# helenypzhang/Subspace-Multimodal-Learning

Measured on AMD Instinct MI355X. Metric: bags/sec fwd+bwd, DeformCrossTransMIL N=10k x 512, higher is better.
Workload: dtype f32

## Files before the change

### include/smml.h

```cpp
#ifndef SMML_H_
#define SMML_H_

#include <stddef.h>

#define SMML_ABI_VERSION 2

#ifdef __cplusplus
extern "C" {
#endif

const char* smml_last_error(void);
int smml_abi_version(void);
int smml_device_check(int device);
void* smml_event_create(void);
int smml_event_destroy(void* ev);
int smml_event_record(void* ev, void* stream);
int smml_event_elapsed_ms(void* start, void* stop, float* ms);

int smml_gemm_f32(const float* A, const float* B, float* C, const float* bias, const float* residual,
                  int M, int N, int K, long long sam, long long sak, long long sbk, long long sbn,
                  long long ldc, long long ldr, int nb0, int nb1, long long sa0, long long sa1,
                  long long sb0, long long sb1, long long sc0, long long sc1, long long sbias0,
                  long long sbias1, int bias_mode, int rows_per_bias, long long bias_ld, int act,
                  int splitk, int accumulate, float alpha, float beta, void* stream);
size_t smml_gemm_f32_det_workspace_bytes(int M, int N, int nb0, int nb1, int splitk);
int smml_gemm_f32_det(const float* A, const float* B, float* C, const float* bias, const float* residual,
                      int M, int N, int K, long long sam, long long sak, long long sbk, long long sbn,
                      long long ldc, long long ldr, int nb0, int nb1, long long sa0, long long sa1,
                      long long sb0, long long sb1, long long sc0, long long sc1, long long sbias0,
                      long long sbias1, int bias_mode, int rows_per_bias, long long bias_ld, int act,
                      int splitk, int accumulate, float alpha, float beta, void* workspace, size_t workspace_bytes,
                      void* stream);
void smml_gemm_force_generic(int on);
void smml_gemm_set_mode(int mode);
int smml_gemm_get_mode(void);
void smml_gemm_set_small_tile(int v);

int smml_gemm_b16(const void* A, const void* B, void* C, const float* bias, int M, int N, int K, long long lda, long long ldb,
                  long long ldc, int trans, int out_bf16, int splitk, void* stream);
void smml_gemm_b16_set_tile(int mode);
void smml_gemm_b16_set_slice_major(int on);
int smml_gemm_b16_batched(const void* A, const void* B, void* C, const float* bias, int M, int N, int K, long long lda, long long ldb,
                          long long ldc, int trans, int out_bf16, int splitk, int nb, long long sa, long long sb, long long sc, void* stream);

int smml_grouped_pointwise_applies(int groups, int cin_g, int cout_g);
int smml_grouped_pointwise_fwd_f32(const float* x, const float* w, float* y, long long rows, int groups, int cin_g, int cout_g, void* stream);
int smml_grouped_pointwise_dx_f32(const float* dy, const float* w, float* dx, long long rows, int groups, int cin_g, int cout_g, void* stream);
size_t smml_grouped_pointwise_dw_workspace_bytes(long long rows, int groups, int cin_g, int cout_g);
int smml_grouped_pointwise_dw_f32(const float* dy, const float* x, float* dw, long long rows, int groups, int cin_g, int cout_g,
                                  void* workspace, size_t workspace_bytes, void* stream);

int smml_layernorm_fwd_f32(const float* x, const float* gamma, const float* beta, float* y, float* mean,
                           float* rstd, long long R, int C, float eps, void* stream);
int smml_layernorm_bwd_f32(const float* x, const float* dy, const float* gamma, const float* mean,
                           const float* rstd, float* dx, float* dgamma, float* dbeta, long long R, int C,
                           long long rows_per_dy, float dy_scale, int accumulate_dx, void* stream);
size_t smml_layernorm_bwd_det_workspace_bytes(long long R, int C);
int smml_layernorm_bwd_det_f32(const float* x, const float* dy, const float* gamma, const float* mean,
                               const float* rstd, float* dx, float* dgamma, float* dbeta, long long R, int C,
                               long long rows_per_dy, float dy_scale, int accumulate_dx, void* workspace,
                               size_t workspace_bytes, void* stream);

int smml_colsum_f32(const float* x, float* out, int nb, long long R, int C, float scale, void* stream);
size_t smml_colsum_det_workspace_bytes(int nb, long long R, int C);
int smml_colsum_det_f32(const float* x, float* out, int nb, long long R, int C, float scale, void* workspace,
                        size_t workspace_bytes, void* stream);

int smml_orth_loss_f32(const float* P, const float* Ph, const float* G, const float* Gh, const float* dloss, float* loss,
                       float* dP, float* dPh, float* dG, float* dGh, int B, int D, float gamma, void* stream);

int smml_batchloss_tail_f32(const float* go, const float* gv, const float* dloss, float* loss, float* dgo, float* dgv, int R, int nv,
                            float n_total, void* stream);

int smml_relu_bwd_f32(const float* dy, const float* y, float* dx, long long n, void* stream);

int smml_offsets_out_len(int s, int ks, int r);
int smml_offsets_fwd_f32(const float* q, const float* w0, const float* b0, const float* w2, float* vgrid,
                         float* vs, int B, int Hh, int Ww, int G, int dg, int ks, int r, int posdim,
                         float offset_scale, void* stream);
size_t smml_offsets_bwd_workspace_bytes(int B, int Hh, int Ww, int G, int dg, int ks, int r, int posdim);
int smml_offsets_bwd_f32(const float* q, const float* w0, const float* b0, const float* w2,
                         const float* dvgrid, const float* dvs, float* dq, float* dw0, float* db0,
                         float* dw2, void* workspace, size_t workspace_bytes, int B, int Hh, int Ww, int G, int dg,
                         int ks, int r, int posdim, float offset_scale, int accumulate_dq, void* stream);

int smml_bilinear_sample_fwd_f32(const float* x, const float* vs, float* kv, int B, int Hh, int Ww, int G,
// ... 260 lines not shown
```

### subspace-multimodal-learning_amd/csrc/rowops.hip

```cpp
#include <algorithm>
#include "smml_common.h"

namespace {

constexpr int MAXV = 16;

__global__ __launch_bounds__(256) void layernorm_fwd_kernel(const float* __restrict__ x, const float* __restrict__ gamma,
                                                            const float* __restrict__ beta, float* __restrict__ y,
                                                            float* __restrict__ mean, float* __restrict__ rstd, long long R,
                                                            int C, float eps) {
  const int lane = threadIdx.x & 63;
  const long long row = (long long)blockIdx.x * 4 + (threadIdx.x >> 6);
  if (row >= R) return;
  const float* xr = x + row * C;
  float v[MAXV];
  float s = 0.f;
  const int nv = (C + 63) >> 6;
#pragma unroll
  for (int i = 0; i < MAXV; ++i) {
    if (i < nv) {
      const int c = lane + 64 * i;
      v[i] = (c < C) ? xr[c] : 0.f;
      s += v[i];
    }
// ... 37 lines not shown
  const int lane = threadIdx.x & 63, wave = threadIdx.x >> 6, hl = lane & 31, half = lane >> 5;
  const bool low = hl < 16;
  const float4 gm = *reinterpret_cast<const float4*>(gamma + 4 * hl), bt = *reinterpret_cast<const float4*>(beta + 4 * hl);
  const long long stride = (long long)gridDim.x * (8 * U);
  for (long long base = ((long long)blockIdx.x * 4 + wave) * (2 * U); base < R; base += stride) {
    float4 xv[U];
#pragma unroll
    for (int u = 0; u < U; ++u) {
      const long long row = base + 2 * u + half;
      xv[u] = *reinterpret_cast<const float4*>(x + (row < R ? row : R - 1) * C + 4 * hl);
    }
#pragma unroll
    for (int u = 0; u < U; ++u) {
      const long long row = base + 2 * u + half;
      const float4 own = xv[u];
      const float4 oth = make_float4(__shfl_xor(own.x, 16), __shfl_xor(own.y, 16), __shfl_xor(own.z, 16), __shfl_xor(own.w, 16));
      const float4 lo = low ? own : oth, hi = low ? oth : own;
      const float mu = row128_sum((0.f + lo.x) + hi.x, (0.f + lo.y) + hi.y, (0.f + lo.z) + hi.z, (0.f + lo.w) + hi.w) / (float)C;
      const float4 dl = make_float4(lo.x - mu, lo.y - mu, lo.z - mu, lo.w - mu);
      const float4 dh = make_float4(hi.x - mu, hi.y - mu, hi.z - mu, hi.w - mu);
      const float ss = row128_sum(fmaf(dh.x, dh.x, dl.x * dl.x), fmaf(dh.y, dh.y, dl.y * dl.y), fmaf(dh.z, dh.z, dl.z * dl.z),
                                  fmaf(dh.w, dh.w, dl.w * dl.w));
      const float rs = rsqrtf(ss / (float)C + eps);
      if (row < R) {
        const float4 d = low ? dl : dh;
        *reinterpret_cast<float4*>(y + row * C + 4 * hl) = make_float4(fmaf(d.x * rs, gm.x, bt.x), fmaf(d.y * rs, gm.y, bt.y),
                                                                       fmaf(d.z * rs, gm.z, bt.z), fmaf(d.w * rs, gm.w, bt.w));
        if (hl == 0) { mean[row] = mu; rstd[row] = rs; }
      }
    }
  }
}

__global__ __launch_bounds__(256) void layernorm_bwd_kernel(const float* __restrict__ x, const float* __restrict__ dy,
                                                            const float* __restrict__ gamma, const float* __restrict__ mean,
                                                            const float* __restrict__ rstd, float* __restrict__ dx,
                                                            float* __restrict__ dgamma, float* __restrict__ dbeta,
                                                            long long R, int C, long long rows_per_dy, float dy_scale,
                                                            int accumulate_dx, float* __restrict__ part) {
  __shared__ float red[2][4][64 * MAXV];
  const int lane = threadIdx.x & 63, wave = threadIdx.x >> 6;
  const int nv = (C + 63) >> 6;
  float ag[MAXV], ab[MAXV], gm[MAXV];
#pragma unroll
  for (int i = 0; i < MAXV; ++i) {
    ag[i] = 0.f; ab[i] = 0.f;
    const int c = lane + 64 * i;
    gm[i] = (i < nv && c < C) ? gamma[c] : 0.f;
  }
  for (long long row = (long long)blockIdx.x * 4 + wave; row < R; row += (long long)gridDim.x * 4) {
    const float* xr = x + row * C;
    const float* dr = dy + (row / rows_per_dy) * C;
    const float mu = mean[row], rs = rstd[row];
    float xh[MAXV], gd[MAXV];
    float s1 = 0.f, s2 = 0.f;
#pragma unroll
    for (int i = 0; i < MAXV; ++i) {
      if (i < nv) {
        const int c = lane + 64 * i;
        const bool ok = c < C;
        const float d = ok ? dr[c] * dy_scale : 0.f;
        xh[i] = ok ? (xr[c] - mu) * rs : 0.f;
        gd[i] = d * gm[i];
        s1 += gd[i];
        s2 += gd[i] * xh[i];
        ag[i] += d * xh[i];
        ab[i] += d;
      }
    }
    s1 = wave_sum(s1) / (float)C;
    s2 = wave_sum(s2) / (float)C;
    float* dxr = dx + row * C;
#pragma unroll
    for (int i = 0; i < MAXV; ++i) {
      if (i < nv) {
        const int c = lane + 64 * i;
        if (c < C) {
          const float v = rs * (gd[i] - s1 - xh[i] * s2);
          dxr[c] = accumulate_dx ? dxr[c] + v : v;
        }
      }
    }
  }
#pragma unroll
  for (int i = 0; i < MAXV; ++i) {
    if (i < nv) { red[0][wave][lane + 64 * i] = ag[i]; red[1][wave][lane + 64 * i] = ab[i]; }
  }
  __syncthreads();
  for (int c = threadIdx.x; c < C; c += 256) {
    const float g = red[0][0][c] + red[0][1][c] + red[0][2][c] + red[0][3][c];
    const float b = red[1][0][c] + red[1][1][c] + red[1][2][c] + red[1][3][c];
    if (part) {
      part[((size_t)blockIdx.x * 2 + 0) * C + c] = g;
      part[((size_t)blockIdx.x * 2 + 1) * C + c] = b;
    } else {
      atomicAdd(&dgamma[c], g);
      atomicAdd(&dbeta[c], b);
    }
  }
}

__device__ __forceinline__ float half_sum(float v) {
#pragma unroll
  for (int off = 16; off > 0; off >>= 1) v += __shfl_xor(v, off);
  return v;
}

__global__ __launch_bounds__(256) void layernorm_bwd128_kernel(const float* __restrict__ x, const float* __restrict__ dy,
                                                               const float* __restrict__ gamma, const float* __restrict__ mean,
                                                               const float* __restrict__ rstd, float* __restrict__ dx,
                                                               float* __restrict__ dgamma, float* __restrict__ dbeta,
                                                               long long R, long long rows_per_dy, float dy_scale,
                                                               int accumulate_dx, float* __restrict__ part) {
  constexpr int C = 128;
  __shared__ float red[2][8][C];
  const int lane = threadIdx.x & 63, wave = threadIdx.x >> 6, hl = lane & 31, half = lane >> 5;
  const float4 gm = *reinterpret_cast<const float4*>(gamma + 4 * hl);
  float4 ag = make_float4(0.f, 0.f, 0.f, 0.f), ab = ag;
  const long long stride = (long long)gridDim.x * 16;
  for (long long r0 = ((long long)blockIdx.x * 4 + wave) * 4 + half; r0 < R; r0 += stride) {
    float4 xv[2], dv[2];
    float mu[2], rs[2];
    bool ok[2];
#pragma unroll
    for (int u = 0; u < 2; ++u) {
      const long long row = r0 + 2 * u;
      ok[u] = row < R;
      const long long rr = ok[u] ? row : R - 1;
      xv[u] = *reinterpret_cast<const float4*>(x + rr * C + 4 * hl);
      dv[u] = *reinterpret_cast<const float4*>(dy + (rr / rows_per_dy) * C + 4 * hl);
      mu[u] = mean[rr]; rs[u] = rstd[rr];
    }
#pragma unroll
    for (int u = 0; u < 2; ++u) {
      const float sc = ok[u] ? dy_scale : 0.f;
      const float4 d = make_float4(dv[u].x * sc, dv[u].y * sc, dv[u].z * sc, dv[u].w * sc);
      const float4 xh = make_float4((xv[u].x - mu[u]) * rs[u], (xv[u].y - mu[u]) * rs[u], (xv[u].z - mu[u]) * rs[u],
                                    (xv[u].w - mu[u]) * rs[u]);
      const float4 gd = make_float4(d.x * gm.x, d.y * gm.y, d.z * gm.z, d.w * gm.w);
      float s1 = (gd.x + gd.y) + (gd.z + gd.w);
      float s2 = (gd.x * xh.x + gd.y * xh.y) + (gd.z * xh.z + gd.w * xh.w);
      ag.x += d.x * xh.x; ag.y += d.y * xh.y; ag.z += d.z * xh.z; ag.w += d.w * xh.w;
      ab.x += d.x; ab.y += d.y; ab.z += d.z; ab.w += d.w;
      s1 = half_sum(s1) * (1.f / C);
      s2 = half_sum(s2) * (1.f / C);
      if (ok[u]) {
        float4* dxr = reinterpret_cast<float4*>(dx + (r0 + 2 * u) * C + 4 * hl);
        float4 v = make_float4(rs[u] * (gd.x - s1 - xh.x * s2), rs[u] * (gd.y - s1 - xh.y * s2),
                               rs[u] * (gd.z - s1 - xh.z * s2), rs[u] * (gd.w - s1 - xh.w * s2));
        if (accumulate_dx) { const float4 o = *dxr; v.x += o.x; v.y += o.y; v.z += o.z; v.w += o.w; }
        *dxr = v;
      }
    }
  }
  *reinterpret_cast<float4*>(&red[0][wave * 2 + half][4 * hl]) = ag;
  *reinterpret_cast<float4*>(&red[1][wave * 2 + half][4 * hl]) = ab;
  __syncthreads();
  if (threadIdx.x < C) {
    float g = 0.f, bsum = 0.f;
#pragma unroll
    for (int i = 0; i < 8; ++i) { g += red[0][i][threadIdx.x]; bsum += red[1][i][threadIdx.x]; }
    if (part) {
      part[((size_t)blockIdx.x * 2 + 0) * C + threadIdx.x] = g;
      part[((size_t)blockIdx.x * 2 + 1) * C + threadIdx.x] = bsum;
    } else {
      atomicAdd(&dgamma[threadIdx.x], g);
      atomicAdd(&dbeta[threadIdx.x], bsum);
    }
  }
}

__global__ __launch_bounds__(256) void colsum_kernel(const float* __restrict__ x, float* __restrict__ out, long long R,
                                                     int C, float scale, int rows_per_block, float* __restrict__ part) {
  __shared__ float red[256];
  const int b = blockIdx.y;
  const long long r0 = (long long)blockIdx.x * rows_per_block;
  const long long r1 = min(R, r0 + rows_per_block);
  for (int cb = 0; cb < C; cb += 256) {
    const int ncol = min(256, C - cb);
    int cp = 1;
    while (cp < ncol) cp <<= 1;
    const int rl = 256 / cp;
    const int col = threadIdx.x % cp, rlane = threadIdx.x / cp;
// ... 156 lines not shown
  const float go = dloss[b];
  const float s1 = -copysignf(1.f, c1) * go, s2 = -copysignf(1.f, c2) * go;
  const float s3 = gamma * copysignf(1.f, c3) * go, s4 = gamma * copysignf(1.f, c4) * go, s5 = gamma * copysignf(1.f, c5) * go;
  for (int i = lane; i < D; i += 64) {
    const float a = p[i], c = ph[i], e = g[i], f = gh[i];
    dPh[(long long)b * D + i] = s1 * (a / (np * nh) - c1 * c / (nh * nh)) + s5 * (e / (ng * nh) - c5 * c / (nh * nh));
    dGh[(long long)b * D + i] = s2 * (e / (ng * nk) - c2 * f / (nk * nk)) + s4 * (a / (np * nk) - c4 * f / (nk * nk));
    dP[(long long)b * D + i] = s3 * (e / (np * ng) - c3 * a / (np * np));
    dG[(long long)b * D + i] = s3 * (a / (np * ng) - c3 * e / (ng * ng));
  }
}

}

extern "C" {

int smml_layernorm_fwd_f32(const float* x, const float* gamma, const float* beta, float* y, float* mean, float* rstd,
                           long long R, int C, float eps, void* stream) {
  SMML_REQUIRE(x && gamma && beta && y && mean && rstd, "smml_layernorm_fwd_f32: null pointer");
  SMML_REQUIRE(R > 0 && C > 0 && C <= 64 * MAXV, "smml_layernorm_fwd_f32: need 0 < C <= %d (got %d)", 64 * MAXV, C);
  const bool aligned = ((reinterpret_cast<size_t>(x) | reinterpret_cast<size_t>(y) | reinterpret_cast<size_t>(gamma) |
                         reinterpret_cast<size_t>(beta)) & 15) == 0;
  if (C == 128 && aligned) {
    const long long nb = (R + 8 * LN128_RPT - 1) / (8 * LN128_RPT);
    hipLaunchKernelGGL(layernorm_fwd128_kernel, dim3((unsigned)(nb < 2048 ? nb : 2048)), dim3(256), 0, (hipStream_t)stream, x, gamma,
                       beta, y, mean, rstd, R, eps);
  } else
  hipLaunchKernelGGL(layernorm_fwd_kernel, dim3((unsigned)((R + 3) / 4)), dim3(256), 0, (hipStream_t)stream, x, gamma,
                     beta, y, mean, rstd, R, C, eps);
  SMML_LAUNCH_CHECK("smml_layernorm_fwd_f32");
  return SMML_OK;
}

int smml_layernorm_bwd_f32(const float* x, const float* dy, const float* gamma, const float* mean, const float* rstd,
                           float* dx, float* dgamma, float* dbeta, long long R, int C, long long rows_per_dy,
                           float dy_scale, int accumulate_dx, void* stream) {
  SMML_REQUIRE(x && dy && gamma && mean && rstd && dx && dgamma && dbeta, "smml_layernorm_bwd_f32: null pointer");
  SMML_REQUIRE(R > 0 && C > 0 && C <= 64 * MAXV, "smml_layernorm_bwd_f32: need 0 < C <= %d (got %d)", 64 * MAXV, C);
  SMML_REQUIRE(rows_per_dy >= 1, "smml_layernorm_bwd_f32: rows_per_dy must be >= 1");
  const long long nblk = (R + 3) / 4;
  const bool aligned = ((reinterpret_cast<size_t>(x) | reinterpret_cast<size_t>(dy) | reinterpret_cast<size_t>(dx) |
                         reinterpret_cast<size_t>(gamma)) & 15) == 0;
  if (C == 128 && aligned) {
    const long long nb16 = (R + 15) / 16;
    hipLaunchKernelGGL(layernorm_bwd128_kernel, dim3((unsigned)(nb16 < 768 ? nb16 : 768)), dim3(256), 0, (hipStream_t)stream,
                       x, dy, gamma, mean, rstd, dx, dgamma, dbeta, R, rows_per_dy, dy_scale, accumulate_dx, (float*)nullptr);
  } else
  hipLaunchKernelGGL(layernorm_bwd_kernel, dim3((unsigned)(nblk < 1024 ? nblk : 1024)), dim3(256), 0, (hipStream_t)stream,
                     x, dy, gamma, mean, rstd, dx, dgamma, dbeta, R, C, rows_per_dy, dy_scale, accumulate_dx, (float*)nullptr);
  SMML_LAUNCH_CHECK("smml_layernorm_bwd_f32");
  return SMML_OK;
}

int smml_colsum_f32(const float* x, float* out, int nb, long long R, int C, float scale, void* stream) {
  SMML_REQUIRE(x && out && nb > 0 && R > 0 && C > 0, "smml_colsum_f32: bad argument");
  SMML_REQUIRE(nb <= 65535, "smml_colsum_f32: too many batches");
  if ((C & 3) == 0 && C <= 1024 && 256 % (C >> 2) == 0 && ((reinterpret_cast<size_t>(x) & 15) == 0)) {
    const int rl = 256 / (C >> 2);
    long long rpb = std::max<long long>(64LL * rl, (R * nb + 2047) / 2048);
    rpb = (rpb + rl - 1) / rl * rl;
    const long long nb4 = (R + rpb - 1) / rpb;
    hipLaunchKernelGGL(colsum4_kernel, dim3((unsigned)nb4, (unsigned)nb), dim3(256), 0, (hipStream_t)stream, x, out, R, C, scale, (int)rpb, (float*)nullptr);
    SMML_LAUNCH_CHECK("smml_colsum_f32/4");
    return SMML_OK;
  }
  int rows_per_block = 256;
  long long nblk = (R + rows_per_block - 1) / rows_per_block;
  hipLaunchKernelGGL(colsum_kernel, dim3((unsigned)nblk, (unsigned)nb), dim3(256), 0, (hipStream_t)stream, x, out, R, C,
                     scale, rows_per_block, (float*)nullptr);
  SMML_LAUNCH_CHECK("smml_colsum_f32");
  return SMML_OK;
}

static long long layernorm_bwd_det_workgroups(long long R, int C) {
  if (C == 128) { const long long nb16 = (R + 15) / 16; return nb16 < 768 ? nb16 : 768; }
  const long long nblk = (R + 3) / 4;
  return nblk < 1024 ? nblk : 1024;
}

size_t smml_layernorm_bwd_det_workspace_bytes(long long R, int C) {
  if (R <= 0 || C <= 0 || C > 64 * MAXV) return 0;
  return (size_t)layernorm_bwd_det_workgroups(R, C) * 2 * (size_t)C * sizeof(float);
}

int smml_layernorm_bwd_det_f32(const float* x, const float* dy, const float* gamma, const float* mean, const float* rstd,
                               float* dx, float* dgamma, float* dbeta, long long R, int C, long long rows_per_dy,
                               float dy_scale, int accumulate_dx, void* workspace, size_t workspace_bytes, void* stream) {
  SMML_REQUIRE(x && dy && gamma && mean && rstd && dx && dgamma && dbeta && workspace, "smml_layernorm_bwd_det_f32: null pointer");
  SMML_REQUIRE(R > 0 && C > 0 && C <= 64 * MAXV, "smml_layernorm_bwd_det_f32: need 0 < C <= %d (got %d)", 64 * MAXV, C);
  SMML_REQUIRE(rows_per_dy >= 1, "smml_layernorm_bwd_det_f32: rows_per_dy must be >= 1");
  SMML_REQUIRE(workspace_bytes >= smml_layernorm_bwd_det_workspace_bytes(R, C), "smml_layernorm_bwd_det_f32: workspace too small");
  const long long nwg = layernorm_bwd_det_workgroups(R, C);
  float* part = (float*)workspace;
  const bool aligned = ((reinterpret_cast<size_t>(x) | reinterpret_cast<size_t>(dy) | reinterpret_cast<size_t>(dx) |
                         reinterpret_cast<size_t>(gamma)) & 15) == 0;
  if (C == 128 && aligned)
    hipLaunchKernelGGL(layernorm_bwd128_kernel, dim3((unsigned)nwg), dim3(256), 0, (hipStream_t)stream,
                       x, dy, gamma, mean, rstd, dx, dgamma, dbeta, R, rows_per_dy, dy_scale, accumulate_dx, part);
  else
    hipLaunchKernelGGL(layernorm_bwd_kernel, dim3((unsigned)nwg), dim3(256), 0, (hipStream_t)stream,
                       x, dy, gamma, mean, rstd, dx, dgamma, dbeta, R, C, rows_per_dy, dy_scale, accumulate_dx, part);
  SMML_LAUNCH_CHECK("smml_layernorm_bwd_det_f32");
  hipLaunchKernelGGL(slab_reduce_kernel, dim3((unsigned)((2 * C + 31) / 32)), dim3(256), 0, (hipStream_t)stream, part, nwg, (long long)2 * C,
                     dgamma, dbeta, (long long)C, 1);
  SMML_LAUNCH_CHECK("smml_layernorm_bwd_det_f32/reduce");
  return SMML_OK;
}

// ... 66 lines not shown
```

### subspace-multimodal-learning_amd/deform_cross_trans_mil.py

```python
from __future__ import annotations

import math

import torch
from torch import nn

from . import functional as Fh
from .deform_attention import DeformCrossAttention1D, DeformCrossAttention2D


class FusionNet(nn.Module):
    def __init__(self, feature_dim=128):
        super().__init__()
        self.fusion_layer = nn.Linear(feature_dim * 2, feature_dim)

    def forward(self, gene_features, image_features):
        C = self.fusion_layer.out_features
        w = self.fusion_layer.weight
        if image_features.dim() == 3:
            image_features = image_features[:, 0]
        row_bias = Fh.linear(image_features, w[:, C:], self.fusion_layer.bias)
        return Fh.linear(gene_features, w[:, :C], row_bias, rows_per_bias=gene_features.shape[1])


# ... 29 lines not shown
        return Fh.linear(avg, self.dense.weight, self.dense.bias, act=Fh.ACT_TANH)


class DeformCrossTransMIL(nn.Module):
    def __init__(self, args, n_classes=4):
        super().__init__()
        cd = getattr(args, "deform_compute_dtype", None)
        self.fusion_layer = FusionNet(feature_dim=128)
        in_dim = int(getattr(args, "input_path_dim", 1024) or 1024)
        self._fc1 = nn.Sequential(nn.Linear(in_dim, args.path_dim), nn.ReLU())
        self.cls_token = nn.Parameter(torch.randn(1, 1, args.path_dim))
        self.args = args
        self.n_classes = n_classes
        self.layer3 = DeformCrossTransLayer(dim=args.path_dim, grid_hw=getattr(args, "grid_hw", None), compute_dtype=cd,
                                            cpb_table=getattr(args, "deform_cpb_table", False),
                                            cpb_regions_1d=bool(getattr(args, "deform1d_cpb_regions", False)))
        self.norm = nn.LayerNorm(args.path_dim)
        self._fc2 = nn.Linear(args.path_dim, self.n_classes)
        self.pooler = Pooler(args.path_dim)
        self.multimodal_projection = nn.Linear(args.path_dim, self.args.path_dim)
        self._maps_out = None

    def prefetch(self, n_tokens: int) -> None:
        if self.args.attn_dim == 2 and not bool(getattr(self.args, "wrap_pad_to_square", False)):
            self.layer3.attn2d.prefetch_regions(n_tokens)

    def forward(self, path, omic):
        self.prefetch(path.shape[1])
        return self.forward_features(Fh.linear(path.float(), self._fc1[0].weight, self._fc1[0].bias, act=Fh.ACT_RELU), omic)

    def forward_features(self, path, omic):
        omic = omic.float()
        N = path.shape[1]
        h = self.fusion_layer(path, omic)
        vgrid = None
        if self.args.attn_dim == 1:
            B = h.shape[0]
            cls = self.cls_token.expand(B, -1, -1).to(h.device)
            h = torch.cat((cls, h), dim=1)
            pth = torch.cat((cls, path), dim=1)
            h = self.layer3(h, pth, 1, self.args.return_vgrid)
            h = Fh.layer_norm(h[:, :1], self.norm.weight, self.norm.bias, self.norm.eps)[:, 0]
            logits = Fh.linear(h, self._fc2.weight, self._fc2.bias)
        elif self.args.attn_dim == 2:
            pth = path
            side = int(math.ceil(math.sqrt(N)))
            wrap = bool(getattr(self.args, "wrap_pad_to_square", False)) and side * side != N and getattr(self.args, "grid_hw", None) is None
            if wrap:
                add = side * side - N
                h = torch.cat((h, h[:, :add]), dim=1)
                pth = torch.cat((path, path[:, :add]), dim=1)
            if self._maps_out is not None:
                r = self.layer3(h, pth, 2, bool(self.args.return_vgrid), return_attn_maps=self._maps_out[0])
                h, vgrid = r[0], (r[1] if self.args.return_vgrid else None)
                self._maps_out.append(r[-1])
            elif self.args.return_vgrid:
                h, vgrid = self.layer3(h, pth, 2, True)
            else:
                h = self.layer3(h, pth, 2, False)
            if wrap:
                h = h[:, :N]
            avg = Fh.layer_norm_token_mean(h, self.norm.weight, self.norm.bias, self.norm.eps)
            h = Fh.linear(avg, self.pooler.dense.weight, self.pooler.dense.bias, act=Fh.ACT_TANH)
            logits = Fh.linear(h, self._fc2.weight, self._fc2.bias)
        else:
            raise ValueError(f"attn_dim must be 1 or 2 (got {self.args.attn_dim})")
        encoded = Fh.linear(h, self.multimodal_projection.weight, self.multimodal_projection.bias)
        path_grads = None
        if self.args.return_vgrid:
            if vgrid is None:
                raise RuntimeError("return_vgrid requires attn_dim == 2 (the reference raises NameError here, "
                                   "DeformCrossTransMIL.py:158)")
            omic_tiled = Fh.tile_tokens(omic, N)
            return encoded, logits, path_grads, omic_tiled, vgrid
        return encoded, logits, path_grads

    def _maps_check(self):
        if self.args.attn_dim != 2:
            raise ValueError(f"attention_maps needs attn_dim = 2 (got {self.args.attn_dim}): the 1-D branch's default sampler reads the centre "
                             "token for every key, so its attention says nothing about where in the bag the model looked")
# ... 11 lines not shown
```

### subspace-multimodal-learning_amd/functional.py

```python
from __future__ import annotations

import math
import os
from typing import Optional

import ctypes as C_

import torch

from . import _capi as capi

ACT_NONE, ACT_RELU, ACT_TANH = 0, 1, 2
ACT_SIGMOID = 3
ACT_TANH_SIGMOID = 4


DETERMINISTIC = os.environ.get("SMML_DETERMINISTIC", "0") not in ("", "0")


def set_deterministic(on: bool) -> None:
    global DETERMINISTIC
    DETERMINISTIC = bool(on)


# ... 147 lines not shown
    def __enter__(self):
        if self.mode:
            L = capi.lib()
            self.prev = L.smml_gemm_get_mode()
            L.smml_gemm_set_mode(self.mode)

    def __exit__(self, *a):
        if self.mode:
            capi.lib().smml_gemm_set_mode(self.prev)


def _splitk_for(out_rows: int, out_cols: int, k: int, batches: int = 1) -> int:
    tiles = ((out_rows + 127) // 128) * ((out_cols + 63) // 64) * batches
    want = max(1, 1024 // max(tiles, 1))
    return int(max(1, min(want, (k + 255) // 256, 65535 // max(batches, 1))))


def colsum(x2d_or_3d: torch.Tensor, scale: float = 1.0, det: Optional[bool] = None) -> torch.Tensor:
    x = x2d_or_3d
    nb, R, Cc = x.shape
    if DETERMINISTIC if det is None else det:
        L = capi.lib()
        out = torch.empty(nb, Cc, device=x.device, dtype=torch.float32)
        wsb = L.smml_colsum_det_workspace_bytes(nb, R, Cc)
        ws = _scratch(wsb, x.device)
        capi.check(L.smml_colsum_det_f32(capi.fptr(x), capi.fptr(out), nb, R, Cc, float(scale), capi.fptr(ws), wsb, capi.stream()),
                   "colsum (deterministic)")
        return out
    out = _ZEROS.zeros((nb, Cc), x.device)
    capi.check(capi.lib().smml_colsum_f32(capi.fptr(x), capi.fptr(out), nb, R, Cc, float(scale), capi.stream()), "colsum")
    return out


class _Linear(torch.autograd.Function):
    @staticmethod
    def forward(ctx, x, weight, bias, act, rows_per_bias, residual, prec=0):
        x = _c(x); weight = _c(weight)
        ctx.det = DETERMINISTIC
        ctx.prec = 3 if prec == 4 else prec
        K = x.shape[-1]
        M = x.numel() // K
        N = weight.shape[0]
        y = torch.empty(*x.shape[:-1], N, device=x.device, dtype=torch.float32)
        bias_mode = 0
        if bias is not None:
            bias = _c(bias)
            bias_mode = 2 if bias.dim() == 2 else 1
        res = _c(residual) if residual is not None else None
        with _prec(prec):
            _gemm(x, weight, y, M=M, N=N, K=K, sam=K, sak=1, sbk=1, sbn=K, ldc=N, bias=bias, bias_mode=bias_mode,
                  rows_per_bias=rows_per_bias, bias_ld=N, residual=res, ldr=N, act=act)
        ctx.act, ctx.rows_per_bias, ctx.bias_mode = act, rows_per_bias, bias_mode
        ctx.has_res = residual is not None
        ctx.save_for_backward(x, weight, y if act != ACT_NONE else None)
        return y

    @staticmethod
    def backward(ctx, dy):
        x, weight, y = ctx.saved_tensors
        dy = _c(dy)
        K = x.shape[-1]
        M = x.numel() // K
        N = weight.shape[0]
        dres = dy if ctx.has_res else None
        if ctx.act == ACT_RELU:
            dpre = torch.empty_like(dy)
            capi.check(capi.lib().smml_relu_bwd_f32(capi.fptr(dy), capi.fptr(y), capi.fptr(dpre), dy.numel(),
                                                    capi.stream()), "relu_bwd")
        elif ctx.act == ACT_TANH:
            dpre = dy * (1.0 - y * y)
        elif ctx.act == ACT_SIGMOID:
            dpre = dy * (y * (1.0 - y))
        elif ctx.act == ACT_TANH_SIGMOID:
            yv, yu = y[..., :N // 2], y[..., N // 2:]
            dpre = dy * torch.cat((1.0 - yv * yv, yu * (1.0 - yu)), dim=-1)
        else:
            dpre = dy
        dx = dw = db = None
        with _prec(ctx.prec):
            if ctx.needs_input_grad[0]:
                dx = torch.empty_like(x)
                _gemm(dpre, weight, dx, M=M, N=K, K=N, sam=N, sak=1, sbk=K, sbn=1, ldc=K)
            if ctx.needs_input_grad[1]:
                dw = torch.empty_like(weight) if ctx.det else _zeros_like(weight)
                _gemm(dpre, x, dw, M=N, N=K, K=M, sam=1, sak=N, sbk=K, sbn=1, ldc=K, splitk=_splitk_for(N, K, M), det=ctx.det)
        if ctx.bias_mode and ctx.needs_input_grad[2]:
            if ctx.bias_mode == 1:
                db = colsum(dpre.reshape(1, M, N), det=ctx.det)[0]
            else:
                db = colsum(dpre.reshape(M // ctx.rows_per_bias, ctx.rows_per_bias, N), det=ctx.det)
        return dx, dw, db, None, None, dres, None


def linear(x, weight, bias=None, act: int = ACT_NONE, rows_per_bias: int = 1, residual=None, prec: int = 0):
    if act == ACT_TANH_SIGMOID and weight.shape[0] % 2:
        raise ValueError(f"linear: ACT_TANH_SIGMOID splits the output columns in halves, got an odd N = {weight.shape[0]}")
    return _Linear.apply(x, weight, bias, act, rows_per_bias, residual, prec)


class _DualLinearRelu(torch.autograd.Function):
    @staticmethod
    def forward(ctx, x, w0, b0, w1, b1):
        x = _c(x)
        ctx.det = DETERMINISTIC
        K = x.shape[-1]
        M = x.numel() // K
        N = w0.shape[0]
        w = torch.stack((_c(w0), _c(w1)))
        b = torch.stack((_c(b0), _c(b1)))
        y = torch.empty(2, *x.shape[:-1], N, device=x.device, dtype=torch.float32)
        _gemm(x, w, y, M=M, N=N, K=K, sam=K, sak=1, sbk=1, sbn=K, ldc=N, bias=b, bias_mode=1, act=ACT_RELU, nb1=2, sa1=0,
              sb1=N * K, sc1=M * N, sbias1=N)
        ctx.save_for_backward(x, y)
        return y[0], y[1]

    @staticmethod
    def backward(ctx, dy0, dy1):
        x, y = ctx.saved_tensors
        K = x.shape[-1]
        M = x.numel() // K
        N = y.shape[-1]
        L = capi.lib()
        dpre = torch.empty_like(y)
        for i, dy in enumerate((dy0, dy1)):
            capi.check(L.smml_relu_bwd_f32(capi.fptr(_c(dy)), capi.fptr(y[i]), capi.fptr(dpre[i]), dy.numel(), capi.stream()), "relu_bwd")
        dx = None
        if ctx.needs_input_grad[0]:
            raise RuntimeError("dual_linear_relu: the shared input is a bag of features (no gradient path is built)")
        dw = torch.empty(2, N, K, device=x.device, dtype=torch.float32) if ctx.det else _ZEROS.zeros((2, N, K), x.device)
        _gemm(dpre, x, dw, M=N, N=K, K=M, sam=1, sak=N, sbk=K, sbn=1, ldc=K, nb1=2, sa1=M * N, sb1=0, sc1=N * K,
# ... 931 lines not shown
        dx = dw = None
        if ctx.streaming and _al16(dy):
            L = capi.lib()
            if ctx.needs_input_grad[0]:
                dx = torch.empty_like(x)
                capi.check(L.smml_grouped_pointwise_dx_f32(capi.fptr(dy), capi.fptr(w), capi.fptr(dx), M, G, cin_g, cout_g, capi.stream()),
                           "grouped_pointwise dx")
            if ctx.needs_input_grad[1]:
                dw = torch.empty_like(w)
                wsb = L.smml_grouped_pointwise_dw_workspace_bytes(M, G, cin_g, cout_g)
                ws = _scratch(wsb, dy.device)
                capi.check(L.smml_grouped_pointwise_dw_f32(capi.fptr(dy), capi.fptr(x), capi.fptr(dw), M, G, cin_g, cout_g, capi.fptr(ws), wsb,
                                                           capi.stream()), "grouped_pointwise dw")
                dw = dw.reshape(ctx.wshape)
            return dx, dw, None
        if ctx.needs_input_grad[0]:
            dx = torch.empty_like(x)
            _gemm(dy, w, dx, M=M, N=cin_g, K=cout_g, sam=Cout, sak=1, sbk=cin_g, sbn=1, ldc=Cin, nb1=G,
                  sa1=cout_g, sb1=cout_g * cin_g, sc1=cin_g)
        if ctx.needs_input_grad[1]:
            dw = torch.empty_like(w) if ctx.det else _zeros_like(w)
            _gemm(dy, x, dw, M=cout_g, N=cin_g, K=M, sam=1, sak=Cout, sbk=Cin, sbn=1, ldc=cin_g, nb1=G,
                  sa1=cout_g, sb1=cin_g, sc1=cout_g * cin_g, splitk=_splitk_for(cout_g, cin_g, M, G), det=ctx.det)
            dw = dw.reshape(ctx.wshape)
        return dx, dw, None


def grouped_pointwise(x, weight, groups: int = 1):
    return _GroupedPointwise.apply(x, weight, groups)


class _LayerNorm(torch.autograd.Function):
    @staticmethod
    def forward(ctx, x, gamma, beta, eps, token_mean):
        x = _c(x); gamma = _c(gamma); beta = _c(beta)
        Cc = x.shape[-1]
        R = x.numel() // Cc
        y = torch.empty_like(x)
        mean = torch.empty(R, device=x.device, dtype=torch.float32)
        rstd = torch.empty(R, device=x.device, dtype=torch.float32)
        capi.check(capi.lib().smml_layernorm_fwd_f32(capi.fptr(x), capi.fptr(gamma), capi.fptr(beta), capi.fptr(y),
                                                     capi.fptr(mean), capi.fptr(rstd), R, Cc, float(eps),
                                                     capi.stream()), "layernorm_fwd")
        ctx.token_mean = token_mean
        ctx.det = DETERMINISTIC
        ctx.save_for_backward(x, gamma, mean, rstd)
        if token_mean:
            assert x.dim() == 3
            return colsum(y, 1.0 / x.shape[1], det=ctx.det)
        return y

    @staticmethod
    def backward(ctx, dy):
        x, gamma, mean, rstd = ctx.saved_tensors
        dy = _c(dy)
        Cc = x.shape[-1]
        R = x.numel() // Cc
        dx = torch.empty_like(x)
        dg = _zeros_like(gamma)
        db = _zeros_like(gamma)
        rows_per_dy, scale = (x.shape[1], 1.0 / x.shape[1]) if ctx.token_mean else (1, 1.0)
        if ctx.det:
            L = capi.lib()
            wsb = L.smml_layernorm_bwd_det_workspace_bytes(R, Cc)
            ws = _scratch(wsb, x.device)
            capi.check(L.smml_layernorm_bwd_det_f32(capi.fptr(x), capi.fptr(dy), capi.fptr(gamma), capi.fptr(mean), capi.fptr(rstd),
                                                    capi.fptr(dx), capi.fptr(dg), capi.fptr(db), R, Cc, rows_per_dy, float(scale), 0,
                                                    capi.fptr(ws), wsb, capi.stream()), "layernorm_bwd (deterministic)")
            return dx, dg, db, None, None
        capi.check(capi.lib().smml_layernorm_bwd_f32(capi.fptr(x), capi.fptr(dy), capi.fptr(gamma), capi.fptr(mean),
                                                     capi.fptr(rstd), capi.fptr(dx), capi.fptr(dg), capi.fptr(db), R, Cc,
                                                     rows_per_dy, float(scale), 0, capi.stream()), "layernorm_bwd")
        return dx, dg, db, None, None


def layer_norm(x, gamma, beta, eps: float = 1e-5):
    return _LayerNorm.apply(x, gamma, beta, eps, False)


def layer_norm_token_mean(x, gamma, beta, eps: float = 1e-5):
    return _LayerNorm.apply(x, gamma, beta, eps, True)


class GradFork:
    __slots__ = ("dq",)

    def __init__(self):
        self.dq = None


class _Offsets(torch.autograd.Function):
    @staticmethod
    def forward(ctx, q, w0, b0, w2, groups, ks, r, posdim, offset_scale, fork=None):
        ctx.fork = fork
        q = _c(q); w0c = _c(w0); b0c = _c(b0); w2c = _c(w2)
        B, Hh, Ww, inner = q.shape
        dg = inner // groups
        L = capi.lib()
        tw = L.smml_offsets_out_len(Ww, ks, r)
        th = L.smml_offsets_out_len(Hh, ks, r) if posdim == 2 else 1
        if th <= 0 or tw <= 0:
            raise RuntimeError("token grid too small for the offset convolution")
        J = th * tw
        vgrid = torch.empty((B * groups, 2, th, tw) if posdim == 2 else (B * groups, tw), device=q.device,
                            dtype=torch.float32)
        vs = torch.empty(B * groups, J, posdim, device=q.device, dtype=torch.float32)
        capi.check(L.smml_offsets_fwd_f32(capi.fptr(q), capi.fptr(w0c), capi.fptr(b0c), capi.fptr(w2c),
                                          capi.fptr(vgrid), capi.fptr(vs), B, Hh, Ww, groups, dg, ks, r, posdim,
                                          float(offset_scale), capi.stream()), "offsets_fwd")
        ctx.cfg = (groups, ks, r, posdim, float(offset_scale))
        ctx.save_for_backward(q, w0c, b0c, w2c)
        return vgrid, vs

    @staticmethod
# ... 652 lines not shown
            Hh, Ww = int(grid_hw[0]), int(grid_hw[1])
            vsc = _c(vs.detach())
            if tuple(vsc.shape) != (B * groups, J, 2):
                raise ValueError(f"vs of shape {tuple(vsc.shape)}: expected {(B * groups, J, 2)}")
            patch_map = torch.empty(B, groups, Hh, Ww, device=lse.device, dtype=torch.float32)
            capi.check(L.smml_attn_splat_f32(capi.fptr(key_mass), capi.fptr(vsc), capi.fptr(patch_map), B, H, groups, J, Hh, Ww, capi.stream()),
                       "attn_splat")
            res["patch_map"] = patch_map
        if dense:
            res["attn"] = attn
    return res


class _TokenMean(torch.autograd.Function):
    @staticmethod
    def forward(ctx, x):
        x = _c(x)
        ctx.n = x.shape[1]
        return colsum(x, 1.0 / x.shape[1], det=DETERMINISTIC)

    @staticmethod
    def backward(ctx, dy):
        return (dy / ctx.n).unsqueeze(1).expand(-1, ctx.n, -1).contiguous()


def token_mean(x):
    return _TokenMean.apply(x)


class _TileTokens(torch.autograd.Function):
    @staticmethod
    def forward(ctx, v, n):
        ctx.det = DETERMINISTIC
        return v.unsqueeze(1).repeat(1, n, 1)

    @staticmethod
    def backward(ctx, dy):
        return colsum(_c(dy), det=ctx.det), None


def tile_tokens(v, n: int):
    out = _TileTokens.apply(v, n)
    out._smml_compact = v
    return out


class _Gram(torch.autograd.Function):

    @staticmethod
    def forward(ctx, x):
        x = _c(x)
        nb, R, K = x.shape
        det = DETERMINISTIC
        g = (torch.empty if det else torch.zeros)(nb, R, R, device=x.device, dtype=torch.float32)
        splitk = int(max(1, min((K + 255) // 256, 1024 // max(nb, 1), 65535 // nb)))
        _gemm(x, x, g, M=R, N=R, K=K, sam=K, sak=1, sbk=1, sbn=K, ldc=R, nb0=nb, sa0=R * K, sb0=R * K, sc0=R * R,
              splitk=splitk, det=det)
        ctx.save_for_backward(x)
        return g

    @staticmethod
    def backward(ctx, dg):
        (x,) = ctx.saved_tensors
        nb, R, K = x.shape
        s = _c(dg + dg.transpose(1, 2))
        dx = torch.empty_like(x)
        _gemm(s, x, dx, M=R, N=K, K=R, sam=R, sak=1, sbk=K, sbn=1, ldc=K, nb0=nb, sa0=R * R, sb0=R * K, sc0=R * K)
# ... 335 lines not shown
```

Baseline: 1270.

## Fuse layernorm with token mean and accumulate forked gradients in place

Adds a 128-column layernorm kernel that reduces straight into the per-bag token mean, so the full normalized tensor is never written out and no separate column-sum pass runs. Adds a GradSum mechanism: when one tensor feeds both a linear and a layernorm, the first backward parks its gradient and the second accumulates into it (GEMM residual or accumulate_dx), so autograd no longer does an extra add over the large activation gradient. The backward kernel now preloads the old dx, and tile_tokens uses expand instead of repeat. The parking relies on a private autograd task-id hook and adds bookkeeping complexity.

After: 1283 (median of 6 runs). 1.01x the previous value.

```diff
diff --git a/include/smml.h b/include/smml.h
--- a/include/smml.h
+++ b/include/smml.h
@@ -52,6 +52,11 @@
 
 int smml_layernorm_fwd_f32(const float* x, const float* gamma, const float* beta, float* y, float* mean,
                            float* rstd, long long R, int C, float eps, void* stream);
+int smml_layernorm_fwd_mean_f32(const float* x, const float* gamma, const float* beta, float* mean, float* rstd, float* out, int nb,
+                                long long n, int C, float eps, void* stream);
+size_t smml_layernorm_fwd_mean_det_workspace_bytes(int nb, long long n, int C);
+int smml_layernorm_fwd_mean_det_f32(const float* x, const float* gamma, const float* beta, float* mean, float* rstd, float* out, int nb,
+                                    long long n, int C, float eps, void* workspace, size_t workspace_bytes, void* stream);
 int smml_layernorm_bwd_f32(const float* x, const float* dy, const float* gamma, const float* mean,
                            const float* rstd, float* dx, float* dgamma, float* dbeta, long long R, int C,
                            long long rows_per_dy, float dy_scale, int accumulate_dx, void* stream);
diff --git a/subspace-multimodal-learning_amd/csrc/rowops.hip b/subspace-multimodal-learning_amd/csrc/rowops.hip
--- a/subspace-multimodal-learning_amd/csrc/rowops.hip
+++ b/subspace-multimodal-learning_amd/csrc/rowops.hip
@@ -93,6 +93,63 @@
   }
 }
 
+__global__ __launch_bounds__(256) void layernorm_fwd128_mean_kernel(const float* __restrict__ x, const float* __restrict__ gamma,
+                                                                    const float* __restrict__ beta, float* __restrict__ mean,
+                                                                    float* __restrict__ rstd, float* __restrict__ out, long long n,
+                                                                    float eps, float scale, int rows_per_chunk, float* __restrict__ part) {
+  constexpr int C = 128, U = LN128_RPT;
+  __shared__ float red[8][C];
+  const int lane = threadIdx.x & 63, wave = threadIdx.x >> 6, hl = lane & 31, half = lane >> 5;
+  const int b = blockIdx.y;
+  const bool low = hl < 16;
+  const float4 gm = *reinterpret_cast<const float4*>(gamma + 4 * hl), bt = *reinterpret_cast<const float4*>(beta + 4 * hl);
+  const long long lo_row = (long long)blockIdx.x * rows_per_chunk, hi_row = min(n, lo_row + rows_per_chunk);
+  const float* xb = x + (long long)b * n * C;
+  float4 acc = make_float4(0.f, 0.f, 0.f, 0.f);
+  for (long long base = lo_row + wave * (2 * U); base < hi_row; base += 8 * U) {
+    float4 xv[U];
+#pragma unroll
+    for (int u = 0; u < U; ++u) {
+      const long long row = base + 2 * u + half;
+      xv[u] = *reinterpret_cast<const float4*>(xb + (row < hi_row ? row : hi_row - 1) * C + 4 * hl);
+    }
+#pragma unroll
+    for (int u = 0; u < U; ++u) {
+      const long long row = base + 2 * u + half;
+      const float4 own = xv[u];
+      const float4 oth = make_float4(__shfl_xor(own.x, 16), __shfl_xor(own.y, 16), __shfl_xor(own.z, 16), __shfl_xor(own.w, 16));
+      const float4 lo = low ? own : oth, hi = low ? oth : own;
+      const float mu = row128_sum((0.f + lo.x) + hi.x, (0.f + lo.y) + hi.y, (0.f + lo.z) + hi.z, (0.f + lo.w) + hi.w) / (float)C;
+      const float4 dl = make_float4(lo.x - mu, lo.y - mu, lo.z - mu, lo.w - mu);
+      const float4 dh = make_float4(hi.x - mu, hi.y - mu, hi.z - mu, hi.w - mu);
+      const float ss = row128_sum(fmaf(dh.x, dh.x, dl.x * dl.x), fmaf(dh.y, dh.y, dl.y * dl.y), fmaf(dh.z, dh.z, dl.z * dl.z),
+                                  fmaf(dh.w, dh.w, dl.w * dl.w));
+      const float rs = rsqrtf(ss / (float)C + eps);
+      if (row < hi_row) {
+        const float4 d = low ? dl : dh;
+        acc.x += fmaf(d.x * rs, gm.x, bt.x); acc.y += fmaf(d.y * rs, gm.y, bt.y);
+        acc.z += fmaf(d.z * rs, gm.z, bt.z); acc.w += fmaf(d.w * rs, gm.w, bt.w);
+        if (hl == 0) { mean[(long long)b * n + row] = mu; rstd[(long long)b * n + row] = rs; }
+      }
+    }
+  }
+  *reinterpret_cast<float4*>(&red[wave * 2 + half][4 * hl]) = acc;
+  __syncthreads();
+  if (threadIdx.x < C) {
+    float t = 0.f;
+#pragma unroll
+    for (int i = 0; i < 8; ++i) t += red[i][threadIdx.x];
+    t *= scale;
+    if (part) part[((size_t)blockIdx.x * gridDim.y + b) * C + threadIdx.x] = t;
+    else atomicAdd(&out[(long long)b * C + threadIdx.x], t);
+  }
+}
+
+__device__ __forceinline__ float add_rn(float a, float b) {
+#pragma clang fp contract(off)
+  return a + b;
+}
+
 __global__ __launch_bounds__(256) void layernorm_bwd_kernel(const float* __restrict__ x, const float* __restrict__ dy,
                                                             const float* __restrict__ gamma, const float* __restrict__ mean,
                                                             const float* __restrict__ rstd, float* __restrict__ dx,
@@ -138,7 +195,7 @@
         const int c = lane + 64 * i;
         if (c < C) {
           const float v = rs * (gd[i] - s1 - xh[i] * s2);
-          dxr[c] = accumulate_dx ? dxr[c] + v : v;
+          dxr[c] = accumulate_dx ? add_rn(dxr[c], v) : v;
         }
       }
     }
@@ -167,24 +224,25 @@
   return v;
 }
 
+constexpr int LN128_BWD_RPT = 2;
 __global__ __launch_bounds__(256) void layernorm_bwd128_kernel(const float* __restrict__ x, const float* __restrict__ dy,
                                                                const float* __restrict__ gamma, const float* __restrict__ mean,
                                                                const float* __restrict__ rstd, float* __restrict__ dx,
                                                                float* __restrict__ dgamma, float* __restrict__ dbeta,
                                                                long long R, long long rows_per_dy, float dy_scale,
                                                                int accumulate_dx, float* __restrict__ part) {
-  constexpr int C = 128;
+  constexpr int C = 128, U = LN128_BWD_RPT;
   __shared__ float red[2][8][C];
   const int lane = threadIdx.x & 63, wave = threadIdx.x >> 6, hl = lane & 31, half = lane >> 5;
   const float4 gm = *reinterpret_cast<const float4*>(gamma + 4 * hl);
   float4 ag = make_float4(0.f, 0.f, 0.f, 0.f), ab = ag;
-  const long long stride = (long long)gridDim.x * 16;
-  for (long long r0 = ((long long)blockIdx.x * 4 + wave) * 4 + half; r0 < R; r0 += stride) {
-    float4 xv[2], dv[2];
-    float mu[2], rs[2];
-    bool ok[2];
-#pragma unroll
-    for (int u = 0; u < 2; ++u) {
+  const long long stride = (long long)gridDim.x * (8 * U);
+  for (long long r0 = ((long long)blockIdx.x * 4 + wave) * (2 * U) + half; r0 < R; r0 += stride) {
+    float4 xv[U], dv[U];
+    float mu[U], rs[U];
+    bool ok[U];
+#pragma unroll
+    for (int u = 0; u < U; ++u) {
       const long long row = r0 + 2 * u;
       ok[u] = row < R;
       const long long rr = ok[u] ? row : R - 1;
@@ -192,8 +250,16 @@
       dv[u] = *reinterpret_cast<const float4*>(dy + (rr / rows_per_dy) * C + 4 * hl);
       mu[u] = mean[rr]; rs[u] = rstd[rr];
     }
-#pragma unroll
-    for (int u = 0; u < 2; ++u) {
+    float4 ov[U];
+    if (accumulate_dx) {
+#pragma unroll
+      for (int u = 0; u < U; ++u) {
+        ov[u] = make_float4(0.f, 0.f, 0.f, 0.f);
+        if (ok[u]) ov[u] = *reinterpret_cast<const float4*>(dx + (r0 + 2 * u) * C + 4 * hl);
+      }
+    }
+#pragma unroll
+    for (int u = 0; u < U; ++u) {
       const float sc = ok[u] ? dy_scale : 0.f;
       const float4 d = make_float4(dv[u].x * sc, dv[u].y * sc, dv[u].z * sc, dv[u].w * sc);
       const float4 xh = make_float4((xv[u].x - mu[u]) * rs[u], (xv[u].y - mu[u]) * rs[u], (xv[u].z - mu[u]) * rs[u],
@@ -209,7 +275,10 @@
         float4* dxr = reinterpret_cast<float4*>(dx + (r0 + 2 * u) * C + 4 * hl);
         float4 v = make_float4(rs[u] * (gd.x - s1 - xh.x * s2), rs[u] * (gd.y - s1 - xh.y * s2),
                                rs[u] * (gd.z - s1 - xh.z * s2), rs[u] * (gd.w - s1 - xh.w * s2));
-        if (accumulate_dx) { const float4 o = *dxr; v.x += o.x; v.y += o.y; v.z += o.z; v.w += o.w; }
+        if (accumulate_dx) {
+          const float4 o = ov[u];
+          v = make_float4(add_rn(v.x, o.x), add_rn(v.y, o.y), add_rn(v.z, o.z), add_rn(v.w, o.w));
+        }
         *dxr = v;
       }
     }
@@ -432,6 +501,61 @@
   return SMML_OK;
 }
 
+static long long layernorm_mean_rows_per_chunk(long long n) {
+  if (n <= 1024) return 512;
+  const long long want = (n + 2047) / 2048;
+  return want <= 64 ? 64 : (want + 31) / 32 * 32;
+}
+
+static int layernorm_mean_launch(const char* fn, const float* x, const float* gamma, const float* beta, float* mean, float* rstd,
+                                 float* out, int nb, long long n, int C, float eps, float* part, void* stream) {
+  SMML_REQUIRE(x && gamma && beta && mean && rstd && out, "%s: null pointer", fn);
+  SMML_REQUIRE(nb > 0 && nb <= 65535 && n > 0, "%s: need 0 < nb <= 65535 bags of n > 0 rows", fn);
+  SMML_REQUIRE(C == 128, "%s: the fused token mean has a 128-column kernel only (got C = %d)", fn, C);
+  SMML_REQUIRE(((reinterpret_cast<size_t>(x) | reinterpret_cast<size_t>(gamma) | reinterpret_cast<size_t>(beta)) & 15) == 0,
+               "%s: x, gamma and beta must be 16-byte aligned", fn);
+  const long long rpc = layernorm_mean_rows_per_chunk(n), chunks = (n + rpc - 1) / rpc;
+  SMML_REQUIRE(rpc <= 2147483647LL && chunks <= 2147483647LL, "%s: too many rows", fn);
+  hipLaunchKernelGGL(layernorm_fwd128_mean_kernel, dim3((unsigned)chunks, (unsigned)nb), dim3(256), 0, (hipStream_t)stream, x, gamma, beta,
+                     mean, rstd, out, n, eps, 1.f / (float)n, (int)rpc, part);
+  return SMML_OK;
+}
+
+int smml_layernorm_fwd_mean_f32(const float* x, const float* gamma, const float* beta, float* mean, float* rstd, float* out, int nb,
+                                long long n, int C, float eps, void* stream) {
+  if (int rc = layernorm_mean_launch("smml_layernorm_fwd_mean_f32", x, gamma, beta, mean, rstd, out, nb, n, C, eps, nullptr, stream)) return rc;
+  SMML_LAUNCH_CHECK("smml_layernorm_fwd_mean_f32");
+  return SMML_OK;
+}
+
+size_t smml_layernorm_fwd_mean_det_workspace_bytes(int nb, long long n, int C) {
+  if (nb <= 0 || n <= 0 || C != 128) return 0;
+  const long long rpc = layernorm_mean_rows_per_chunk(n);
+  return (size_t)((n + rpc - 1) / rpc) * (size_t)nb * (size_t)C * sizeof(float);
+}
+
+int smml_layernorm_fwd_mean_det_f32(const float* x, const float* gamma, const float* beta, float* mean, float* rstd, float* out, int nb,
+                                    long long n, int C, float eps, void* workspace, size_t workspace_bytes, void* stream) {
+  SMML_REQUIRE(workspace && out, "smml_layernorm_fwd_mean_det_f32: null pointer");
+  SMML_REQUIRE(nb > 0 && n > 0 && C == 128, "smml_layernorm_fwd_mean_det_f32: need nb > 0, n > 0 and C = 128");
+  SMML_REQUIRE(workspace_bytes >= smml_layernorm_fwd_mean_det_workspace_bytes(nb, n, C), "smml_layernorm_fwd_mean_det_f32: workspace too small");
+  const long long rpc = layernorm_mean_rows_per_chunk(n), chunks = (n + rpc - 1) / rpc;
+  float* part = chunks == 1 ? out : (float*)workspace;
+  if (int rc = layernorm_mean_launch("smml_layernorm_fwd_mean_det_f32", x, gamma, beta, mean, rstd, out, nb, n, C, eps, part, stream)) return rc;
+  SMML_LAUNCH_CHECK("smml_layernorm_fwd_mean_det_f32");
+  if (chunks == 1) return SMML_OK;
+  const long long ncols = (long long)nb * C;
+  hipLaunchKernelGGL(slab_reduce_kernel, dim3((unsigned)((ncols + 31) / 32)), dim3(256), 0, (hipStream_t)stream, part, chunks, ncols, out,
+                     out, ncols, 0);
+  SMML_LAUNCH_CHECK("smml_layernorm_fwd_mean_det_f32/reduce");
+  return SMML_OK;
+}
+
+static long long layernorm_bwd128_workgroups(long long R) {
+  const long long nb = (R + 8 * LN128_BWD_RPT - 1) / (8 * LN128_BWD_RPT);
+  return nb < 768 ? nb : 768;
+}
+
 int smml_layernorm_bwd_f32(const float* x, const float* dy, const float* gamma, const float* mean, const float* rstd,
                            float* dx, float* dgamma, float* dbeta, long long R, int C, long long rows_per_dy,
                            float dy_scale, int accumulate_dx, void* stream) {
@@ -442,8 +566,7 @@
   const bool aligned = ((reinterpret_cast<size_t>(x) | reinterpret_cast<size_t>(dy) | reinterpret_cast<size_t>(dx) |
                          reinterpret_cast<size_t>(gamma)) & 15) == 0;
   if (C == 128 && aligned) {
-    const long long nb16 = (R + 15) / 16;
-    hipLaunchKernelGGL(layernorm_bwd128_kernel, dim3((unsigned)(nb16 < 768 ? nb16 : 768)), dim3(256), 0, (hipStream_t)stream,
+    hipLaunchKernelGGL(layernorm_bwd128_kernel, dim3((unsigned)layernorm_bwd128_workgroups(R)), dim3(256), 0, (hipStream_t)stream,
                        x, dy, gamma, mean, rstd, dx, dgamma, dbeta, R, rows_per_dy, dy_scale, accumulate_dx, (float*)nullptr);
   } else
   hipLaunchKernelGGL(layernorm_bwd_kernel, dim3((unsigned)(nblk < 1024 ? nblk : 1024)), dim3(256), 0, (hipStream_t)stream,
@@ -473,7 +596,7 @@
 }
 
 static long long layernorm_bwd_det_workgroups(long long R, int C) {
-  if (C == 128) { const long long nb16 = (R + 15) / 16; return nb16 < 768 ? nb16 : 768; }
+  if (C == 128) return layernorm_bwd128_workgroups(R);
   const long long nblk = (R + 3) / 4;
   return nblk < 1024 ? nblk : 1024;
 }
diff --git a/subspace-multimodal-learning_amd/deform_cross_trans_mil.py b/subspace-multimodal-learning_amd/deform_cross_trans_mil.py
--- a/subspace-multimodal-learning_amd/deform_cross_trans_mil.py
+++ b/subspace-multimodal-learning_amd/deform_cross_trans_mil.py
@@ -85,7 +85,14 @@
     def forward_features(self, path, omic):
         omic = omic.float()
         N = path.shape[1]
+        side = int(math.ceil(math.sqrt(N)))
+        wrap = bool(getattr(self.args, "wrap_pad_to_square", False)) and side * side != N and getattr(self.args, "grid_hw", None) is None
+        joined = self.args.attn_dim == 2 and not wrap and Fh.GRAD_SUM and torch.is_grad_enabled()
+        if joined and path.requires_grad:
+            path = Fh.grad_sum(path.view_as(path))
         h = self.fusion_layer(path, omic)
+        if joined:
+            Fh.grad_sum(h)
         vgrid = None
         if self.args.attn_dim == 1:
             B = h.shape[0]
@@ -97,8 +104,6 @@
             logits = Fh.linear(h, self._fc2.weight, self._fc2.bias)
         elif self.args.attn_dim == 2:
             pth = path
-            side = int(math.ceil(math.sqrt(N)))
-            wrap = bool(getattr(self.args, "wrap_pad_to_square", False)) and side * side != N and getattr(self.args, "grid_hw", None) is None
             if wrap:
                 add = side * side - N
                 h = torch.cat((h, h[:, :add]), dim=1)
diff --git a/subspace-multimodal-learning_amd/functional.py b/subspace-multimodal-learning_amd/functional.py
--- a/subspace-multimodal-learning_amd/functional.py
+++ b/subspace-multimodal-learning_amd/functional.py
@@ -203,9 +203,48 @@
     return out
 
 
+GRAD_SUM = os.environ.get("SMML_GRAD_SUM", "1") != "0"
+
+
+class GradSum:
+    __slots__ = ("parked", "owner", "task")
+
+    def __init__(self):
+        self.parked = self.owner = self.task = None
+
+    @staticmethod
+    def _task():
+        fn = getattr(torch._C, "_current_graph_task_id", None)
+        t = fn() if fn is not None else -1
+        return None if t < 0 else t
+
+    def take(self, who: str, like: torch.Tensor) -> Optional[torch.Tensor]:
+        t, task = self.parked, self._task()
+        if t is None or self.owner == who or task is None or self.task != task:
+            return None
+        self.parked = self.owner = self.task = None
+        ok = t.dtype == torch.float32 and t.is_contiguous() and t.shape == like.shape and t.device == like.device and t.data_ptr() % 16 == 0
+        return t if ok else None
+
+    def park(self, who: str, t: torch.Tensor) -> None:
+        task = self._task()
+        self.parked, self.owner, self.task = (t, who, task) if task is not None else (None, None, None)
+
+
+def grad_sum(t: torch.Tensor) -> torch.Tensor:
+    if GRAD_SUM and t.requires_grad:
+        t._smml_grad_sum = GradSum()
+    return t
+
+
+def _fork_of(t) -> Optional[GradSum]:
+    return getattr(t, "_smml_grad_sum", None) if (GRAD_SUM and t is not None) else None
+
+
 class _Linear(torch.autograd.Function):
     @staticmethod
-    def forward(ctx, x, weight, bias, act, rows_per_bias, residual, prec=0):
+    def forward(ctx, x, weight, bias, act, rows_per_bias, residual, prec=0, xfork=None, rfork=None):
+        ctx.xfork, ctx.rfork = xfork, rfork
         x = _c(x); weight = _c(weight)
         ctx.det = DETERMINISTIC
         ctx.prec = 3 if prec == 4 else prec
@@ -234,6 +273,8 @@
         M = x.numel() // K
         N = weight.shape[0]
         dres = dy if ctx.has_res else None
+        if dres is not None and ctx.rfork is not None and ctx.needs_input_grad[5]:
+            ctx.rfork.park("linear", dres)
         if ctx.act == ACT_RELU:
             dpre = torch.empty_like(dy)
             capi.check(capi.lib().smml_relu_bwd_f32(capi.fptr(dy), capi.fptr(y), capi.fptr(dpre), dy.numel(),
@@ -250,8 +291,14 @@
         dx = dw = db = None
         with _prec(ctx.prec):
             if ctx.needs_input_grad[0]:
-                dx = torch.empty_like(x)
-                _gemm(dpre, weight, dx, M=M, N=K, K=N, sam=N, sak=1, sbk=K, sbn=1, ldc=K)
+                parked = ctx.xfork.take("linear", x) if ctx.xfork is not None else None
+                if parked is not None:
+                    _gemm(dpre, weight, parked, M=M, N=K, K=N, sam=N, sak=1, sbk=K, sbn=1, ldc=K, residual=parked, ldr=K)
+                else:
+                    dx = torch.empty_like(x)
+                    _gemm(dpre, weight, dx, M=M, N=K, K=N, sam=N, sak=1, sbk=K, sbn=1, ldc=K)
+                    if ctx.xfork is not None:
+                        ctx.xfork.park("linear", dx)
             if ctx.needs_input_grad[1]:
                 dw = torch.empty_like(weight) if ctx.det else _zeros_like(weight)
                 _gemm(dpre, x, dw, M=N, N=K, K=M, sam=1, sak=N, sbk=K, sbn=1, ldc=K, splitk=_splitk_for(N, K, M), det=ctx.det)
@@ -260,13 +307,13 @@
                 db = colsum(dpre.reshape(1, M, N), det=ctx.det)[0]
             else:
                 db = colsum(dpre.reshape(M // ctx.rows_per_bias, ctx.rows_per_bias, N), det=ctx.det)
-        return dx, dw, db, None, None, dres, None
+        return dx, dw, db, None, None, dres, None, None, None
 
 
 def linear(x, weight, bias=None, act: int = ACT_NONE, rows_per_bias: int = 1, residual=None, prec: int = 0):
     if act == ACT_TANH_SIGMOID and weight.shape[0] % 2:
         raise ValueError(f"linear: ACT_TANH_SIGMOID splits the output columns in halves, got an odd N = {weight.shape[0]}")
-    return _Linear.apply(x, weight, bias, act, rows_per_bias, residual, prec)
+    return _Linear.apply(x, weight, bias, act, rows_per_bias, residual, prec, _fork_of(x), _fork_of(residual))
 
 
 class _DualLinearRelu(torch.autograd.Function):
@@ -1264,21 +1311,25 @@
 
 class _LayerNorm(torch.autograd.Function):
     @staticmethod
-    def forward(ctx, x, gamma, beta, eps, token_mean):
+    def forward(ctx, x, gamma, beta, eps, token_mean, fork=None):
+        ctx.fork = fork
         x = _c(x); gamma = _c(gamma); beta = _c(beta)
         Cc = x.shape[-1]
         R = x.numel() // Cc
-        y = torch.empty_like(x)
         mean = torch.empty(R, device=x.device, dtype=torch.float32)
         rstd = torch.empty(R, device=x.device, dtype=torch.float32)
-        capi.check(capi.lib().smml_layernorm_fwd_f32(capi.fptr(x), capi.fptr(gamma), capi.fptr(beta), capi.fptr(y),
-                                                     capi.fptr(mean), capi.fptr(rstd), R, Cc, float(eps),
-                                                     capi.stream()), "layernorm_fwd")
         ctx.token_mean = token_mean
         ctx.det = DETERMINISTIC
         ctx.save_for_backward(x, gamma, mean, rstd)
         if token_mean:
             assert x.dim() == 3
+            if Cc == 128 and _al16(x, gamma, beta):
+                return _layernorm_mean128(x, gamma, beta, mean, rstd, float(eps), ctx.det)
+        y = torch.empty_like(x)
+        capi.check(capi.lib().smml_layernorm_fwd_f32(capi.fptr(x), capi.fptr(gamma), capi.fptr(beta), capi.fptr(y),
+                                                     capi.fptr(mean), capi.fptr(rstd), R, Cc, float(eps),
+                                                     capi.stream()), "layernorm_fwd")
+        if token_mean:
             return colsum(y, 1.0 / x.shape[1], det=ctx.det)
         return y
 
@@ -1288,7 +1339,10 @@
         dy = _c(dy)
         Cc = x.shape[-1]
         R = x.numel() // Cc
-        dx = torch.empty_like(x)
+        fork = ctx.fork if ctx.needs_input_grad[0] else None
+        parked = fork.take("norm", x) if fork is not None else None
+        acc = parked is not None
+        dx = parked if acc else torch.empty_like(x)
         dg = _zeros_like(gamma)
         db = _zeros_like(gamma)
         rows_per_dy, scale = (x.shape[1], 1.0 / x.shape[1]) if ctx.token_mean else (1, 1.0)
@@ -1297,21 +1351,40 @@
             wsb = L.smml_layernorm_bwd_det_workspace_bytes(R, Cc)
             ws = _scratch(wsb, x.device)
             capi.check(L.smml_layernorm_bwd_det_f32(capi.fptr(x), capi.fptr(dy), capi.fptr(gamma), capi.fptr(mean), capi.fptr(rstd),
-                                                    capi.fptr(dx), capi.fptr(dg), capi.fptr(db), R, Cc, rows_per_dy, float(scale), 0,
+                                                    capi.fptr(dx), capi.fptr(dg), capi.fptr(db), R, Cc, rows_per_dy, float(scale), int(acc),
                                                     capi.fptr(ws), wsb, capi.stream()), "layernorm_bwd (deterministic)")
-            return dx, dg, db, None, None
-        capi.check(capi.lib().smml_layernorm_bwd_f32(capi.fptr(x), capi.fptr(dy), capi.fptr(gamma), capi.fptr(mean),
-                                                     capi.fptr(rstd), capi.fptr(dx), capi.fptr(dg), capi.fptr(db), R, Cc,
-                                                     rows_per_dy, float(scale), 0, capi.stream()), "layernorm_bwd")
-        return dx, dg, db, None, None
+        else:
+            capi.check(capi.lib().smml_layernorm_bwd_f32(capi.fptr(x), capi.fptr(dy), capi.fptr(gamma), capi.fptr(mean),
+                                                         capi.fptr(rstd), capi.fptr(dx), capi.fptr(dg), capi.fptr(db), R, Cc,
+                                                         rows_per_dy, float(scale), int(acc), capi.stream()), "layernorm_bwd")
+        if fork is not None and not acc:
+            fork.park("norm", dx)
+        return (None if acc else dx), dg, db, None, None, None
+
+
+def _layernorm_mean128(x, gamma, beta, mean, rstd, eps: float, det: bool) -> torch.Tensor:
+    L = capi.lib()
+    nb, n, Cc = x.shape
+    if det:
+        out = torch.empty(nb, Cc, device=x.device, dtype=torch.float32)
+        wsb = L.smml_layernorm_fwd_mean_det_workspace_bytes(nb, n, Cc)
+        ws = _scratch(wsb, x.device)
+        capi.check(L.smml_layernorm_fwd_mean_det_f32(capi.fptr(x), capi.fptr(gamma), capi.fptr(beta), capi.fptr(mean), capi.fptr(rstd),
+                                                     capi.fptr(out), nb, n, Cc, eps, capi.fptr(ws), wsb, capi.stream()),
+                   "layernorm_fwd_mean (deterministic)")
+        return out
+    out = _ZEROS.zeros((nb, Cc), x.device)
+    capi.check(L.smml_layernorm_fwd_mean_f32(capi.fptr(x), capi.fptr(gamma), capi.fptr(beta), capi.fptr(mean), capi.fptr(rstd),
+                                             capi.fptr(out), nb, n, Cc, eps, capi.stream()), "layernorm_fwd_mean")
+    return out
 
 
 def layer_norm(x, gamma, beta, eps: float = 1e-5):
-    return _LayerNorm.apply(x, gamma, beta, eps, False)
+    return _LayerNorm.apply(x, gamma, beta, eps, False, _fork_of(x))
 
 
 def layer_norm_token_mean(x, gamma, beta, eps: float = 1e-5):
-    return _LayerNorm.apply(x, gamma, beta, eps, True)
+    return _LayerNorm.apply(x, gamma, beta, eps, True, None)
 
 
 class GradFork:
@@ -2030,7 +2103,7 @@
     @staticmethod
     def forward(ctx, v, n):
         ctx.det = DETERMINISTIC
-        return v.unsqueeze(1).repeat(1, n, 1)
+        return v.unsqueeze(1).expand(-1, n, -1)
 
     @staticmethod
     def backward(ctx, dy):
```
